# ZhangYY12345/aswStereoMatch

Hardware: AMD Instinct MI355X
Metric: disparity Mpix/s, 1920x1080 D=128 classic bilateral ASW (computeAdaptiveWeight) (higher is better)
Workload: dtype f64; 1 GPU; 1920x1080 D=128 win=15 bilateral, 8 frames/GPU/step resident in HBM, cost volume kept; candidates=129, parallelism=frames sharded, no collective, ranks=1, backend=none

## Files before the change

aswstereomatch_amd/csrc/asw_internal.h:

```cpp
#pragma once
#include <hip/hip_runtime.h>
#include <stddef.h>
#include <stdint.h>

#include <map>
#include <string>
#include <vector>

#include "../../include/asw_mi355x.h"

#define ASW_HIP_TRY(expr)                                  \
    do {                                                   \
        hipError_t _e = (expr);                            \
        if (_e != hipSuccess) {                            \
            asw_note_hip_error(_e, #expr, __FILE__, __LINE__); \
            return ASW_ERR_HIP;                            \
        }                                                  \
    } while (0)

void asw_note_hip_error(hipError_t e, const char* what, const char* file, int line);

struct DevBuf {
    void* p = nullptr;
    size_t cap = 0;
// ... 86 lines not shown
    const uint8_t* gL;
    const uint8_t* gR;
    int H, W, win, minD, nD;
    const int4* taps;
    const float* lut;
    int ntaps;
    int flip;
    float* vol;
    float* disp;
    double* partE;
    float* partD;
    int max_slices;
    int c_begin = 0;
    int resume = 0;
    int out_slice = -1;
};
int bilateral_xq_candidates(int nwave);
constexpr int XQ_LUT_SCALE_LOG2 = 60;
bool bilateral_xq_lut_ok(const float* lut, size_t n);
int launch_bilateral_xq(hipStream_t s, hipStream_t s_border, int nwave, const uint8_t* gL, const uint8_t* gR, int H, int W, int minD,
                        const int4* cells, const float* lut, float* vol, double* bestE, float* bestD, float* disp, bool right = false);
int launch_bilateral(hipStream_t s, const BilateralLaunch& a);
int launch_merge_slices(hipStream_t s, const double* partE, const float* partD, int nz, size_t plane, float* disp);
int bilateral_lds_row_stride(int win);

int launch_scharr_x(hipStream_t s, const uint8_t* img, int H, int W, int pad, short* grad );
size_t similarity_parts_words(int H, int W, int numD);
int launch_similarity(hipStream_t s, const uint8_t* L, const uint8_t* R, const short* gL, const short* gR, int H, int W,
                      int minD, int numD, double regularity, double thresC, double thresG, float* cost, uint32_t* ord_scratch,
                      float2* scales);
int launch_pad_reflect(hipStream_t s, const float* src, int n, int H, int W, int h, float* dst);
int launch_slice_scales(hipStream_t s, const float* vol, int n, size_t plane, uint32_t* ord_scratch , float2* scales);
int launch_u8_scale(hipStream_t s, const uint8_t* img, size_t nbytes, uint32_t* ord_scratch , float2* scale1);
int launch_guide_scales_lr(hipStream_t s, const uint8_t* ref_img, const uint8_t* shifted_img, int H, int W, int minD, int numD,
                           int disp_type, uint32_t* ord_scratch, int* colmm_scratch , float2* scales );

struct NccLaunch {
    const uint8_t* gref;
// ... 151 lines not shown
```

aswstereomatch_amd/csrc/asw_methods.hip:

```cpp
#include <limits.h>
#include <math.h>
#include <stdio.h>
#include <stdlib.h>
#include <string.h>

#include <mutex>
#include <utility>
#include <vector>

#include "asw_internal.h"
#include "asw_host.h"

static int check_direction(int disparity_type)
{
    return disparity_type == ASW_DISPARITY_LEFT || disparity_type == ASW_DISPARITY_RIGHT ? ASW_OK : ASW_ERR_BAD_ARGUMENT;
}

static int ensure_outputs(Frame* f, int planes, bool keep_volume, bool volume_needed = false)
{
    const size_t plane = (size_t)f->rows * f->cols;
    ASW_TRY(f->disp.ensure(plane * 4));
    f->vol_floats = 0;
    if (keep_volume || volume_needed) ASW_TRY(f->vol.ensure(plane * planes * 4));
    if (keep_volume) f->vol_floats = plane * planes;
// ... 164 lines not shown
    a.H = H; a.W = W; a.win = mp.win; a.minD = mp.minD; a.nD = nD;
    a.taps = ctx->bil.taps.as<int4>(); a.lut = ctx->bil.lut.as<float>(); a.ntaps = ctx->bil.ntaps;
    a.vol = keep_volume ? f->vol.as<float>() : nullptr;
    a.disp = f->disp.as<float>();
    a.partE = nullptr; a.partD = nullptr; a.max_slices = 0;
    const bool xq_fits = flip ? (W - 1) / 64 * 64 + mp.minD <= W - 1 : mp.minD <= 48;
    const int xq_waves = nD >= bilateral_xq_candidates(8) ? 8 : 4;
    const bool use_xq = !direct8 && mp.win == 15 && nD >= bilateral_xq_candidates(xq_waves) && mp.minD >= 0 && xq_fits && W >= 64 &&
                        ctx->bil.xq_lut_ok && ctx->tune.bilateral_xq != 0;
    const size_t plane = (size_t)H * W;
    if (use_xq) {
        a.max_slices = 2;
        ASW_TRY(slice_scratch(ctx, a.max_slices, plane, &a.partE, &a.partD));
        a.c_begin = bilateral_xq_candidates(xq_waves);
        const bool tail = nD > a.c_begin;
        ASW_TRY(agg_begin(ctx));
        ASW_HIP_TRY(hipEventRecord(ctx->aux_ev[0], ctx->stream));
        ASW_HIP_TRY(hipStreamWaitEvent(ctx->aux[0], ctx->aux_ev[0], 0));
        ASW_TRY(launch_bilateral_xq(ctx->stream, ctx->aux[0], xq_waves, a.gL, a.gR, H, W, mp.minD, ctx->bil.cells.as<int4>(), ctx->bil.lut_xq.as<float>(), a.vol,
                                    a.partE, a.partD, tail ? nullptr : a.disp, flip != 0));
        ASW_HIP_TRY(hipEventRecord(ctx->aux_ev[1], ctx->aux[0]));
        if (tail) {
            ASW_HIP_TRY(hipStreamWaitEvent(ctx->aux[1], ctx->aux_ev[0], 0));
            a.out_slice = 1;
            ASW_TRY(launch_bilateral(ctx->aux[1], a));
            ASW_HIP_TRY(hipEventRecord(ctx->aux_ev[2], ctx->aux[1]));
            ASW_HIP_TRY(hipStreamWaitEvent(ctx->stream, ctx->aux_ev[2], 0));
        }
        ASW_HIP_TRY(hipStreamWaitEvent(ctx->stream, ctx->aux_ev[1], 0));
        if (tail) ASW_TRY(launch_merge_slices(ctx->stream, a.partE, a.partD, 2, plane, a.disp));
        return agg_end(ctx, tail ? 4 : 2);
    }
    if (plane <= (size_t)1 << 20) {
        a.max_slices = 8;
        ASW_TRY(slice_scratch(ctx, a.max_slices, plane, &a.partE, &a.partD));
    }
    ASW_TRY(agg_begin(ctx));
    ASW_TRY(launch_bilateral(ctx->stream, a));
    return agg_end(ctx, 1);
}

static int run_bilateral_classic(asw_ctx* ctx, Frame* f, const MatchParams& mp, bool keep_volume)
{
    return run_bilateral(ctx, f, mp, keep_volume, false);
}
// ... 724 lines not shown
```

aswstereomatch_amd/csrc/k_bilateral.hip:

```cpp
#include <stdlib.h>

#include <algorithm>
#include <type_traits>

#include "asw_device.h"
#include "asw_internal.h"

namespace {

constexpr int TW = 64;
constexpr int TH = 4;
constexpr int DCMAX = 16;

struct BilParams {
    int H, W, h, minD, nD, ntaps;
    int flip;
    int cand_per_z;
    int c_begin;
    int resume;
    int out_slice;
};

constexpr __host__ __device__ int round_up(int v, int a) { return (v + a - 1) / a * a; }

struct Layout {
    int h, TR, LW, LWp, RW, RWp, offC, offWR, offWL, offL, offR, total;
    __host__ __device__ constexpr Layout(int h_, int G)
        : h(h_), TR(TH + 2 * h_), LW(TW + 2 * h_), LWp(round_up(TW + 2 * h_, 4)), RW(TW + 2 * h_ + DCMAX - 1),
          RWp(round_up(TW + 2 * h_ + DCMAX - 1, 4)), offC(0), offWR(round_up((TH + 2 * h_) * (TW + 2 * h_) * DCMAX, 16)),
          offWL(offWR + round_up(G * TH * (TW + DCMAX - 1) * 4, 16)),
          offL(offWR + round_up(G * TH * (TW + DCMAX - 1) * 4, 16) + G * TH * TW * 4),
          offR(offWR + round_up(G * TH * (TW + DCMAX - 1) * 4, 16) + G * TH * TW * 4 +
               round_up((TH + 2 * h_) * round_up(TW + 2 * h_, 4), 16)),
          total(offWR + round_up(G * TH * (TW + DCMAX - 1) * 4, 16) + G * TH * TW * 4 +
                round_up((TH + 2 * h_) * round_up(TW + 2 * h_, 4), 16) +
// ... 21 lines not shown
}

template <int DC, int G>
__device__ __forceinline__ void process_chunk(const BilParams& p, const uint8_t* __restrict__ gR,
                                              const int4* __restrict__ taps, const float* __restrict__ lut,
                                              float* __restrict__ vol, const Layout& lay, unsigned char* smem, int c0,
                                              double& bestE, float& bestD)
{
    uint8_t* sL = smem + lay.offL;
    uint8_t* sR = smem + lay.offR;
    uint8_t* sC = smem + lay.offC;
    float* sWR = reinterpret_cast<float*>(smem + lay.offWR);
    float* sWL = reinterpret_cast<float*>(smem + lay.offWL);
    constexpr int SWR = TW + DC - 1;
    const int tid = threadIdx.x, tx = tid & 63, ty = tid >> 6;
    const int x0 = blockIdx.x * TW, y0 = blockIdx.y * TH;
    const int H = p.H, W = p.W, h = lay.h, LW = lay.LW, LWp = lay.LWp, RWp = lay.RWp, TR = lay.TR;
    const int RW = TW + 2 * h + DC - 1;
    const int d0 = p.minD + c0;
    const int sRx0 = max(x0 - h - (d0 + DC - 1), -h);

    __syncthreads();
    for (int i = tid; i < TR * RW; i += 256) {
        int r = i / RW, c = i - r * RW;
        int yy = min(max(y0 - h + r, 0), H - 1), xx = min(max(sRx0 + c, 0), W - 1);
        sR[r * RWp + c] = gR[(size_t)yy * W + (p.flip ? W - 1 - xx : xx)];
    }
    __syncthreads();
    const bool interior = x0 - h - (d0 + DC - 1) >= 0 && x0 + TW + h - d0 <= W;
    const bool interiorC = x0 - h - (d0 + DC - 1) >= 0 && x0 + TW + h <= W;
    for (int i = tid; i < TR * LW; i += 256) {
// ... 92 lines not shown
            load_cost<DC>(myC + tp.x * DC, cw);
            const float* w = myWR + t * (TH * SWR);
#pragma unroll
            for (int dd = 0; dd < DC; dd++) {
                float ab = wl * w[-dd];
                double abd = (double)ab;
                double c = (double)(int)((cw[dd >> 2] >> (8 * (dd & 3))) & 0xffu);
                num[dd] = __builtin_fma(abd, c, num[dd]);
                den[dd] = den[dd] + abd;
            }
        }
        wave_lds_sync();
    }

    const int x = x0 + tx, y = y0 + ty;
    if (x < W && y < H) {
#pragma unroll
        for (int dd = 0; dd < DC; dd++) {
            double E = num[dd] / den[dd];
            if (vol) vol[((size_t)(c0 + dd) * H + y) * W + (p.flip ? W - 1 - x : x)] = (float)E;
            if (E < bestE) {
                bestE = E;
                bestD = (float)(d0 + dd);
            }
        }
    }
}

template <int HH, int G, int WPE>
__global__ __launch_bounds__(256) __attribute__((amdgpu_waves_per_eu(WPE, WPE))) void k_asw_bilateral(
    BilParams p, const uint8_t* __restrict__ gL, const uint8_t* __restrict__ gR, const int4* __restrict__ taps,
    const float* __restrict__ lut, float* __restrict__ vol, float* __restrict__ disp, double* __restrict__ partE,
    float* __restrict__ partD)
{
    extern __shared__ __align__(16) unsigned char smem[];
    const Layout lay(HH > 0 ? HH : p.h, G);
    const int tid = threadIdx.x;
    const int x0 = blockIdx.x * TW, y0 = blockIdx.y * TH;
    const int H = p.H, W = p.W, h = lay.h;

    uint8_t* sL = smem + lay.offL;
    for (int i = tid; i < lay.TR * lay.LW; i += 256) {
        int r = i / lay.LW, c = i - r * lay.LW;
        int yy = min(max(y0 - h + r, 0), H - 1), xx = min(max(x0 - h + c, 0), W - 1);
        sL[r * lay.LWp + c] = gL[(size_t)yy * W + (p.flip ? W - 1 - xx : xx)];
    }

    double bestE = 1.7976931348623157e308;
    float bestD = 0.0f;
    if (p.resume) {
        const int xr = x0 + (tid & 63), yr = y0 + (tid >> 6);
        if (xr < W && yr < H) {
            const size_t o = (size_t)yr * W + (p.flip ? W - 1 - xr : xr);
            bestE = partE[o];
            bestD = partD[o];
        }
    }
    int c0 = p.c_begin + blockIdx.z * p.cand_per_z;
    const int cEnd = min(p.nD, c0 + p.cand_per_z);
    for (; c0 + 16 <= cEnd; c0 += 16) process_chunk<16, G>(p, gR, taps, lut, vol, lay, smem, c0, bestE, bestD);
    if (cEnd - c0 >= 8) { process_chunk<8, G>(p, gR, taps, lut, vol, lay, smem, c0, bestE, bestD); c0 += 8; }
    if (cEnd - c0 >= 4) { process_chunk<4, G>(p, gR, taps, lut, vol, lay, smem, c0, bestE, bestD); c0 += 4; }
    if (cEnd - c0 >= 2) { process_chunk<2, G>(p, gR, taps, lut, vol, lay, smem, c0, bestE, bestD); c0 += 2; }
    if (cEnd - c0 >= 1) { process_chunk<1, G>(p, gR, taps, lut, vol, lay, smem, c0, bestE, bestD); c0 += 1; }

    const int x = x0 + (tid & 63), y = y0 + (tid >> 6);
    if (x < W && y < H) {
        const size_t o = (size_t)y * W + (p.flip ? W - 1 - x : x);
        if (gridDim.z == 1 && p.out_slice < 0) {
            disp[o] = bestD;
        } else {
            const int z = gridDim.z == 1 ? p.out_slice : (int)blockIdx.z;
            partE[(size_t)z * H * W + o] = bestE;
            partD[(size_t)z * H * W + o] = bestD;
        }
    }
}

__global__ __launch_bounds__(256) void k_merge_slices(const double* __restrict__ partE, const float* __restrict__ partD, int nz,
                                                      size_t plane, float* __restrict__ disp)
{
    const size_t o = (size_t)blockIdx.x * blockDim.x + threadIdx.x;
    if (o >= plane) return;
    double best = 1.7976931348623157e308;
    float bd = 0.0f;
    for (int z = 0; z < nz; z++) {
        const double e = partE[(size_t)z * plane + o];
        if (e < best) { best = e; bd = partD[(size_t)z * plane + o]; }
    }
    disp[o] = bd;
}

template <int HH, int G, int WPE = 2>
int launch_t(hipStream_t s, const BilateralLaunch& a)
{
    BilParams p;
    p.H = a.H; p.W = a.W; p.h = a.win / 2; p.minD = a.minD; p.nD = a.nD; p.ntaps = a.ntaps; p.flip = a.flip;
    p.c_begin = a.c_begin; p.resume = a.resume; p.out_slice = a.out_slice;
    if (a.c_begin < 0 || a.c_begin >= a.nD || ((a.resume || a.out_slice >= 0) && !(a.partE && a.partD))) return ASW_ERR_BAD_ARGUMENT;
    const Layout lay(p.h, G);
    if (lay.total > 160 * 1024) return ASW_ERR_BAD_ARGUMENT;
    auto kern = k_asw_bilateral<HH, G, WPE>;
    if (lay.total > 64 * 1024)
        ASW_HIP_TRY(hipFuncSetAttribute(reinterpret_cast<const void*>(kern), hipFuncAttributeMaxDynamicSharedMemorySize, lay.total));
    dim3 grid((a.W + TW - 1) / TW, (a.H + TH - 1) / TH);
    if (a.ntaps % G != 0) return ASW_ERR_BAD_ARGUMENT;
    const int tiles = grid.x * grid.y, chunks16 = (a.nD - a.c_begin + 15) / 16;
    int nz = 1;
    if (a.c_begin == 0 && !a.resume && a.out_slice < 0 && a.partE && a.partD && tiles < 2048) nz = std::min(chunks16, std::min(a.max_slices, (2048 + tiles - 1) / tiles));
    const int chunks_per_z = (chunks16 + nz - 1) / nz;
    nz = (chunks16 + chunks_per_z - 1) / chunks_per_z;
    p.cand_per_z = chunks_per_z * 16;
    grid.z = nz;
    hipLaunchKernelGGL(kern, grid, dim3(256), lay.total, s, p, a.gL, a.gR, a.taps, a.lut, a.vol, a.disp, a.partE, a.partD);
    if (nz > 1) {
        const size_t plane = (size_t)a.H * a.W;
        hipLaunchKernelGGL(k_merge_slices, dim3((unsigned)((plane + 255) / 256)), dim3(256), 0, s, a.partE, a.partD, nz, plane, a.disp);
    }
    ASW_HIP_TRY(hipGetLastError());
    return ASW_OK;
}

}

int bilateral_lds_row_stride(int win) { return TW + 2 * (win / 2); }

int launch_merge_slices(hipStream_t s, const double* partE, const float* partD, int nz, size_t plane, float* disp)
{
    hipLaunchKernelGGL(k_merge_slices, dim3((unsigned)((plane + 255) / 256)), dim3(256), 0, s, partE, partD, nz, plane, disp);
    ASW_HIP_TRY(hipGetLastError());
    return ASW_OK;
}

int launch_bilateral(hipStream_t s, const BilateralLaunch& a)
{
    switch (a.win) {
    case 15: return launch_t<7, 4, 4>(s, a);
    case 35: return launch_t<17, 4, 2>(s, a);
    default: return launch_t<0, 4, 3>(s, a);
    }
}
```

aswstereomatch_amd/csrc/k_bilateral_xq.hip:

```cpp
#include <stdlib.h>

#include <algorithm>
#include <cmath>

#include "asw_device.h"
#include "asw_internal.h"

namespace {

constexpr int HH = 7;
constexpr int KS = 2 * HH + 1;
constexpr int PXW = 64;
constexpr int LWC = PXW + 2 * HH;
constexpr int NSTEP = KS + 3;
constexpr int RING = 5;
constexpr int URI = 3;
constexpr int CROW = 6;
static_assert(KS % URI == 0 && CROW % URI == 0, "whole bodies");
constexpr int NCELLCOL = NSTEP + 3;
constexpr int LW8 = 80;
constexpr int LWP = 80;

template <int NW>
struct XqCfg {
// ... 4 lines not shown
    static constexpr int RWC = NPOS + 2 * HH;
    static constexpr int NFIN = 4 * NJ;
    static constexpr int RW8 = (RWC + 3) / 4 * 4;
    static constexpr int NROWS = (KS + NW - 1) / NW;
    static constexpr int RWP = (RWC + 3) / 4 * 4;
    static constexpr int LROW = RING * PXW + LWP;
    static constexpr int RROW = 2 * NPOS + RWP;
    static constexpr int LGRAY = RING * PXW;
    static constexpr int RGRAY = 2 * NPOS;
    static constexpr int OFF_LB = 0;
    static constexpr int OFF_RB = OFF_LB + KS * LROW * 4;
    static constexpr int OFF_L8 = OFF_RB + KS * RROW * 4;
    static constexpr int OFF_R8 = OFF_L8 + KS * LW8;
    static constexpr int OFF_CELL = OFF_R8 + KS * RW8;
    static constexpr int OFF_E64 = 0;
    static constexpr int OFF_PART = NFIN * PXW * 8;
    static constexpr int LDS_TOTAL = std::max((OFF_CELL + NCELLCOL * KS * 2 + 15) / 16 * 16, OFF_PART + NW * PXW * 12);
    static_assert(LDS_TOTAL <= (NW == 8 ? 80 : 53) * 1024, "two (NW = 8) / three (NW = 4) workgroups per CU");
    static_assert(OFF_RB % 16 == 0 && (LROW * 4) % 16 == 0 && (RROW * 4) % 16 == 0 && (NPOS * 4) % 16 == 0 && (LGRAY * 4) % 16 == 0, "b128 alignment");
    static_assert(NPOS % 64 == 0, "positions are staged in whole wavefront passes");
};
#define XQ_CONSTS(NW)                                                                                                           \
    typedef XqCfg<NW> Cfg;                                                                                                       \
    constexpr int NWAVE = Cfg::NWAVE, NTHR = Cfg::NTHR, NJ = Cfg::NJ, NPOS = Cfg::NPOS, RWC = Cfg::RWC, NFIN = Cfg::NFIN, RW8 = Cfg::RW8,      \
                  NROWS = Cfg::NROWS, LROW = Cfg::LROW, RROW = Cfg::RROW, LGRAY = Cfg::LGRAY, RGRAY = Cfg::RGRAY,               \
                  OFF_LB = Cfg::OFF_LB, OFF_RB = Cfg::OFF_RB, OFF_L8 = Cfg::OFF_L8, OFF_R8 = Cfg::OFF_R8, OFF_CELL = Cfg::OFF_CELL,  \
                  LDS_TOTAL = Cfg::LDS_TOTAL, OFF_E64 = Cfg::OFF_E64, OFF_PART = Cfg::OFF_PART;                                  \
    (void)NWAVE; (void)NTHR; (void)NJ; (void)NPOS; (void)RWC; (void)NFIN; (void)RW8; (void)NROWS; (void)LROW; (void)RROW; (void)LGRAY;  \
    (void)RGRAY; (void)OFF_LB; (void)OFF_RB; (void)OFF_L8; (void)OFF_R8; (void)OFF_CELL; (void)LDS_TOTAL; (void)OFF_E64; (void)OFF_PART;

struct XqParams {
// ... 61 lines not shown
        if (Kn < KS) sWL[ky * LROW + lane] = st.v[rr][0];
#pragma unroll
        for (int r3 = 0; r3 < NPOS / 64; r3++) sWR[ky * RROW + lane + 64 * r3] = st.v[rr][1 + r3];
    }
}

template <int NW>
__device__ __forceinline__ void stage_weights(int Kn, const float* __restrict__ lut, unsigned char* smem, int wave, int lane,
                                              uint32_t ppack)
{
    Staged<NW> st;
    stage_issue<NW>(Kn, lut, smem, wave, lane, ppack, st);
    stage_commit<NW>(Kn, smem, wave, lane, st);
}

template <int NW, int K, bool EDGE, bool WRAPW, bool COMMIT, bool RIGHT>
__device__ __forceinline__ void run_step(unsigned char* smem, int g, int qrel, int qrel2, int xabs, int dbase, int dbase2,
                                         int W, int x0, int posmin, double (&num)[4][4], double (&den)[4][4], int wave, int lane,
                                         const Staged<NW>& st)
{
    XQ_CONSTS(NW)
    constexpr int BLO = K > KS - 1 ? K - (KS - 1) : 0;
    constexpr int BHI = K < 3 ? K : 3;
    constexpr int DLO = 0 - BHI, DHI = 3 - BLO;
    const uint32_t* sLd = reinterpret_cast<const uint32_t*>(smem + OFF_LB) + LGRAY;
    const uint32_t* sRd = reinterpret_cast<const uint32_t*>(smem + OFF_RB) + RGRAY;

    int iL[7], iR[7];
    if constexpr (EDGE) {
#pragma unroll
        for (int dl = DLO; dl <= DHI; dl++) {
            const int lc = min(max(xabs + dl + K - HH, 0), W - 1);
            const int rc = RIGHT ? lc + ((dl > 0 ? dbase2 : dbase) - dl) : lc - ((dl < 0 ? dbase2 : dbase) + dl);
            iL[dl + 3] = min(max(lc - (x0 - HH), 0), LWC - 1);
            iR[dl + 3] = min(max(rc - (posmin - HH), 0), RWC - 1);
        }
    }
    typedef __attribute__((address_space(3))) const unsigned char lds_u8;
    lds_u8* bL = (lds_u8*)smem + OFF_LB + 16 * g;
    lds_u8* bR = (lds_u8*)smem + OFF_RB + 4 * qrel;
    lds_u8* bR2 = (lds_u8*)smem + OFF_RB + 4 * qrel2;
    uint32_t hi0[7];
#pragma unroll
    for (int i = 0; i < 7; i++) asm volatile("v_mov_b32 %0, 0" : "=v"(hi0[i]));
    constexpr int UR = EDGE ? 1 : URI;
    auto rows = [&](int ky0, int nbody) {
#pragma unroll 1
        for (int it = 0; it < nbody; it++) {
#pragma unroll
            for (int u = 0; u < UR; u++) {
                lds_u8* rL = bL + u * 4 * LROW;
                lds_u8* rR = bR + u * 4 * RROW;
                lds_u8* rR2 = bR2 + u * 4 * RROW;
                double c[7];
                if constexpr (!EDGE) {
                    const uint32_t gr = *(const __attribute__((address_space(3))) uint32_t*)(rR + 4 * (RGRAY + K));
                    uint32_t gr2 = gr;
                    if constexpr (WRAPW && (RIGHT ? DHI > 0 : DLO < 0)) gr2 = *(const __attribute__((address_space(3))) uint32_t*)(rR2 + 4 * (RGRAY + K));
                    constexpr int E0 = (K + DLO) & ~3, NQ = (K + DHI - E0 + 4) / 4;
                    static_assert(E0 >= 0 && E0 + 4 * NQ + 4 * 15 <= LWP, "the quads stay inside a tile row");
                    typedef uint32_t u32x4 __attribute__((ext_vector_type(4)));
                    const __attribute__((address_space(3))) u32x4* pl4 = (const __attribute__((address_space(3))) u32x4*)(rL + 4 * (LGRAY + E0));
                    uint32_t glv[4 * NQ];
#pragma unroll
                    for (int i = 0; i < NQ; i++) {
                        u32x4 t = pl4[i];
                        asm("" : "+v"(t));
                        glv[4 * i] = t.x; glv[4 * i + 1] = t.y; glv[4 * i + 2] = t.z; glv[4 * i + 3] = t.w;
                    }
#pragma unroll
                    for (int dl = DLO; dl <= DHI; dl++) c[dl + 3] = cost_sample(glv[K + dl - E0], (RIGHT ? dl > 0 : dl < 0) ? gr2 : gr, hi0[dl + 3]);
                } else {
                    const int ky = ky0 + it * UR + u;
#pragma unroll
                    for (int dl = DLO; dl <= DHI; dl++) c[dl + 3] = cost_sample(sLd[ky * LROW + iL[dl + 3]], sRd[ky * RROW + iR[dl + 3]], hi0[dl + 3]);
                }
                typedef float f32x4 __attribute__((ext_vector_type(4)));
                typedef __attribute__((address_space(3))) const f32x4 lds_f32x4;
                const f32x4 wr4 = *(lds_f32x4*)(rR + 4 * (K & 1) * NPOS);
                typedef float f32x2 __attribute__((ext_vector_type(2)));
                f32x2 wrp[2] = {{wr4.x, wr4.y}, {wr4.z, wr4.w}};
                asm("" : "+v"(wrp[1]));
                f32x2 wr2p[2] = {wrp[0], wrp[1]};
                if constexpr ((WRAPW || EDGE) && (RIGHT ? BLO <= 2 : BHI >= 1)) {
                    const f32x4 w2 = *(lds_f32x4*)(rR2 + 4 * (K & 1) * NPOS);
                    wr2p[0] = f32x2{w2.x, w2.y};
// ... 10 lines not shown
                        const bool w0 = RIGHT ? b < a : a < b, w1 = RIGHT ? b < a + 1 : a + 1 < b;
                        const f32x2 s0 = (w0 ? wr2p : wrp)[b >> 1], s1 = (w1 ? wr2p : wrp)[b >> 1];
                        f32x2 wrb;
                        if (w0 == w1) wrb = (b & 1) ? __builtin_shufflevector(s0, s0, 1, 1) : __builtin_shufflevector(s0, s0, 0, 0);
                        else wrb = f32x2{s0[b & 1], s1[b & 1]};
                        const f32x2 pr = wl2 * wrb;
                        ab[a] = pr.x; ab[a + 1] = pr.y;
                    }
#pragma unroll
                    for (int a = 0; a < 4; a++) {
                        const double abd = (double)ab[a];
                        num[a][b] = __builtin_fma(abd, c[a - b + 3], num[a][b]);
                        den[a][b] = den[a][b] + abd;
                    }
                }
#pragma unroll
                for (int b = BLO; b <= BHI; b++)
                    asm volatile("" :: "v"(num[0][b]), "v"(num[1][b]), "v"(num[2][b]), "v"(num[3][b]),
                                       "v"(den[0][b]), "v"(den[1][b]), "v"(den[2][b]), "v"(den[3][b]) : "memory");
                __builtin_amdgcn_sched_barrier(0);
            }
            bL += UR * 4 * LROW;
            bR += UR * 4 * RROW;
            asm("" : "+v"(bL), "+v"(bR));
            if constexpr (WRAPW || EDGE) {
                bR2 += UR * 4 * RROW;
                asm("" : "+v"(bR2));
            }
        }
    };
    if constexpr (COMMIT) {
        rows(0, CROW / UR);
        stage_commit<NW>(K + 1, smem, wave, lane, st);
        rows(CROW, (KS - CROW) / UR);
    } else {
        rows(0, KS / UR);
    }
}

template <int NW, bool EDGE, bool WRAPW, int ABL, bool RIGHT>
__device__ __forceinline__ void run_all_steps(unsigned char* smem, const float* __restrict__ lut, int wave, int lane,
                                              uint32_t ppack, int g, int qrel, int qrel2, int xabs, int dbase, int dbase2,
                                              int W, int x0, int posmin, double (&num)[4][4], double (&den)[4][4])
{
    Staged<NW> st;
#define ASW_XQ_STEP(KK)                                                                                        \
    if (!(ABL & 1) && (KK) + 1 < NSTEP) {                                                                        \
        if constexpr (EDGE) stage_weights<NW>((KK) + 1, lut, smem, wave, lane, ppack);   \
        else stage_issue<NW>((KK) + 1, lut, smem, wave, lane, ppack, st);                      \
    }                                                                                                           \
    run_step<NW, (KK), EDGE, WRAPW, (!EDGE && !(ABL & 1) && (KK) + 1 < NSTEP), RIGHT>(smem, g, qrel, qrel2, xabs, dbase, dbase2, W, x0, posmin, \
                                                                           num, den, wave, lane, st);          \
    if (!(ABL & 2) || (KK) == NSTEP - 1) __syncthreads();
    ASW_XQ_STEP(0) ASW_XQ_STEP(1) ASW_XQ_STEP(2) ASW_XQ_STEP(3) ASW_XQ_STEP(4) ASW_XQ_STEP(5)
    ASW_XQ_STEP(6) ASW_XQ_STEP(7) ASW_XQ_STEP(8) ASW_XQ_STEP(9) ASW_XQ_STEP(10) ASW_XQ_STEP(11)
    ASW_XQ_STEP(12) ASW_XQ_STEP(13) ASW_XQ_STEP(14) ASW_XQ_STEP(15) ASW_XQ_STEP(16) ASW_XQ_STEP(17)
#undef ASW_XQ_STEP
}

template <int NW, bool EDGE, int ABL, bool RIGHT>
__global__ __launch_bounds__(64 * NW) __attribute__((amdgpu_waves_per_eu(NW == 8 ? 4 : 3, NW == 8 ? 4 : 3))) void k_asw_bilateral_xq(
    XqParams p, const uint8_t* __restrict__ gL, const uint8_t* __restrict__ gR, const int4* __restrict__ cells,
    const float* __restrict__ lut, float* __restrict__ vol, double* __restrict__ bestE, float* __restrict__ bestD,
    float* __restrict__ disp)
{
    XQ_CONSTS(NW)
    __shared__ __align__(16) unsigned char smem[LDS_TOTAL];
    const int tid = threadIdx.x, lane = tid & 63, wave = __builtin_amdgcn_readfirstlane(tid >> 6);
    const int H = p.H, W = p.W;
    const int x0 = (p.tile0 + blockIdx.x) * PXW, y = blockIdx.y;
    const int posmin = RIGHT ? x0 + p.minD : x0 - p.minD - 4 * NJ;

    {
        uint8_t* sL8 = smem + OFF_L8;
        uint8_t* sR8 = smem + OFF_R8;
        uint32_t* sLd = reinterpret_cast<uint32_t*>(smem + OFF_LB) + Cfg::LGRAY;
        uint32_t* sRd = reinterpret_cast<uint32_t*>(smem + OFF_RB) + Cfg::RGRAY;
        for (int i = tid; i < KS * LWC; i += NTHR) {
            const int r = i / LWC, c = i - r * LWC;
            const int yy = min(max(y - HH + r, 0), H - 1), xx = min(max(x0 - HH + c, 0), W - 1);
            const int v = gL[(size_t)yy * W + xx];
            sL8[r * LW8 + c] = (uint8_t)v;
            sLd[r * Cfg::LROW + c] = (uint32_t)v;
        }
        for (int i = tid; i < KS * RWC; i += NTHR) {
            const int r = i / RWC, c = i - r * RWC;
            const int yy = min(max(y - HH + r, 0), H - 1), xx = min(max(posmin - HH + c, 0), W - 1);
            const int v = gR[(size_t)yy * W + xx];
            sR8[r * RW8 + c] = (uint8_t)v;
            sRd[r * Cfg::RROW + c] = (uint32_t)v;
        }
        uint16_t* sCell = reinterpret_cast<uint16_t*>(smem + OFF_CELL);
        for (int i = tid; i < NCELLCOL * KS; i += NTHR) {
            const int4 ci = cells[i];
            sCell[i] = (uint16_t)((uint32_t)(ci.x + 8) | ((uint32_t)(ci.y + 8) << 4) | ((uint32_t)(ci.z >> 8) << 8));
        }
    }
    __syncthreads();

    const int g = (lane & 7) | ((lane >> 2) & 8);
    const int jl = 4 * wave + ((lane >> 3) & 3);
    const int qrel = RIGHT ? 4 * g + 4 * jl : 4 * g + 4 * (NJ - jl);
    const int qrel2 = jl == 0 ? (RIGHT ? 4 * g + 4 * NJ : 4 * g) : qrel;
    const int xabs = x0 + 4 * g;
    const int dbase = p.minD + 4 * jl;
    const int dbase2 = jl == 0 ? p.minD + 4 * NJ : dbase;
    const int pclamp_lo = min(max(0 - posmin, 0), NPOS - 1), pclamp_hi = min(max(W - 1 - posmin, 0), NPOS - 1);
    static_assert(NPOS <= 256, "a clamped position fits a byte");
    uint32_t ppack = 0;
#pragma unroll
    for (int r3 = 0; r3 < NPOS / 64; r3++) ppack |= (uint32_t)min(max(lane + 64 * r3, pclamp_lo), pclamp_hi) << (8 * r3);
    asm volatile("" : "+v"(ppack));

    double num[4][4], den[4][4];
#pragma unroll
    for (int a = 0; a < 4; a++)
#pragma unroll
        for (int b = 0; b < 4; b++) { num[a][b] = 0.0; den[a][b] = 0.0; }

    stage_weights<NW>(0, lut, smem, wave, lane, ppack);
    __syncthreads();
    if (EDGE || wave == 0)
        run_all_steps<NW, EDGE, true, ABL, RIGHT>(smem, lut, wave, lane, ppack, g, qrel, qrel2, xabs, dbase, dbase2, W,
                                                   x0, posmin, num, den);
    else
        run_all_steps<NW, EDGE, false, ABL, RIGHT>(smem, lut, wave, lane, ppack, g, qrel, qrel2, xabs, dbase, dbase2, W,
                                                    x0, posmin, num, den);

    int le = lane;
    asm volatile("" : "+v"(le));
    const int ge = (le & 7) | ((le >> 2) & 8), jle = 4 * wave + ((le >> 3) & 3);
    const int cb = 4 * jle, cb2 = jle == 0 ? 4 * NJ : cb;
    double* sE = reinterpret_cast<double*>(smem + OFF_E64);
#pragma unroll
    for (int a = 0; a < 4; a++)
#pragma unroll
        for (int b = 0; b < 4; b++) {
            const int c = RIGHT ? (b < a ? cb2 : cb) + b - a : (a < b ? cb2 : cb) + a - b;
            sE[c * PXW + 4 * ge + a] = __builtin_ldexp(num[a][b], 954) / __builtin_ldexp(den[a][b], -120);
        }
    __syncthreads();
    const int px = lane, part = wave;
    const int x = x0 + px;
    double be = 1.7976931348623157e308;
    float bd = 0.0f;
    if (x < W) {
        for (int c = 16 * part; c < 16 * part + 16; c++) {
            const double E = sE[c * PXW + px];
            if (vol) vol[((size_t)c * H + y) * W + x] = (float)E;
            if (E < be) { be = E; bd = (float)(p.minD + c); }
        }
    }
    double* sPE = reinterpret_cast<double*>(smem + OFF_PART);
    float* sPD = reinterpret_cast<float*>(smem + OFF_PART + NWAVE * PXW * 8);
    sPE[part * PXW + px] = be;
    sPD[part * PXW + px] = bd;
    __syncthreads();
    if (wave == 0 && x < W) {
        double e = 1.7976931348623157e308;
        float d = 0.0f;
#pragma unroll
        for (int q = 0; q < NWAVE; q++) {
            const double eq = sPE[q * PXW + px];
            if (eq < e) { e = eq; d = sPD[q * PXW + px]; }
        }
        if (disp) {
            disp[(size_t)y * W + x] = d;
        } else {
            bestE[(size_t)y * W + x] = e;
            bestD[(size_t)y * W + x] = d;
        }
    }
}

}

int bilateral_xq_candidates(int nwave) { return 16 * nwave; }

bool bilateral_xq_lut_ok(const float* lut, size_t n)
{
    double mn = 0, mx = 0;
    for (size_t i = 0; i < n; i++) {
        const double v = lut[i];
        if (!(v >= 0)) return false;
        if (v > 0 && (mn == 0 || v < mn)) mn = v;
        if (v > mx) mx = v;
    }
    return mn * mn >= std::ldexp(1.0, -68) && mx * mx < std::ldexp(1.0, 128 - 2 * XQ_LUT_SCALE_LOG2 - 1);
}

namespace {
template <int NW>
int launch_xq_t(hipStream_t s, hipStream_t s_border, const uint8_t* gL, const uint8_t* gR, int H, int W, int minD, const int4* cells,
                const float* lut, float* vol, double* bestE, float* bestD, float* disp, bool right)
{
    const int ntiles = (W + PXW - 1) / PXW;
    const dim3 blk(64 * NW);
    if (right) {
        if ((ntiles - 1) * PXW + minD > W - 1) return ASW_ERR_BAD_ARGUMENT;
        XqParams pe{H, W, minD, 0};
        hipLaunchKernelGGL((k_asw_bilateral_xq<NW, true, 0, true>), dim3(1, H), blk, 0, s_border, pe, gL, gR, cells, lut, vol,
                           bestE, bestD, disp);
        if (ntiles > 1) {
            XqParams pi{H, W, minD, 1};
            hipLaunchKernelGGL((k_asw_bilateral_xq<NW, false, 0, true>), dim3(ntiles - 1, H), blk, 0, s, pi, gL, gR, cells, lut,
                               vol, bestE, bestD, disp);
        }
        ASW_HIP_TRY(hipGetLastError());
        return ASW_OK;
    }
    const int n_int = W >= PXW + HH ? std::min(ntiles, (W - PXW - HH) / PXW + 1) : 0;
#ifdef ASW_XQ_ABLATION
    int abl = 0;
    if (const char* e = getenv("ASW_XQ_ABLATE")) abl = atoi(e) & 3;
    auto ki = abl == 0 ? k_asw_bilateral_xq<NW, false, 0, false> : abl == 1 ? k_asw_bilateral_xq<NW, false, 1, false>
            : abl == 2 ? k_asw_bilateral_xq<NW, false, 2, false> : k_asw_bilateral_xq<NW, false, 3, false>;
#else
    auto ki = k_asw_bilateral_xq<NW, false, 0, false>;
#endif
    auto ke = k_asw_bilateral_xq<NW, true, 0, false>;
    if (n_int > 0) {
        XqParams p{H, W, minD, 0};
        hipLaunchKernelGGL(ki, dim3(n_int, H), blk, 0, s, p, gL, gR, cells, lut, vol, bestE, bestD, disp);
    }
    if (ntiles > n_int) {
        XqParams p{H, W, minD, n_int};
        hipLaunchKernelGGL(ke, dim3(ntiles - n_int, H), blk, 0, s_border, p, gL, gR, cells, lut, vol, bestE, bestD, disp);
    }
    ASW_HIP_TRY(hipGetLastError());
    return ASW_OK;
}
}

int launch_bilateral_xq(hipStream_t s, hipStream_t s_border, int nwave, const uint8_t* gL, const uint8_t* gR, int H, int W, int minD,
                        const int4* cells, const float* lut, float* vol, double* bestE, float* bestD, float* disp, bool right)
{
    if (nwave == 8) return launch_xq_t<8>(s, s_border, gL, gR, H, W, minD, cells, lut, vol, bestE, bestD, disp, right);
    if (nwave == 4) return launch_xq_t<4>(s, s_border, gL, gR, H, W, minD, cells, lut, vol, bestE, bestD, disp, right);
    return ASW_ERR_BAD_ARGUMENT;
}
```

Baseline: 242.8 Mpix/s.

## Fold the last disparity candidate into a spare wavefront of interior xq tiles

With D=128 and 8 waves the xq kernel covers 128 candidates, which leaves one leftover candidate. That candidate used to trigger a full-width launch of the generic bilateral kernel plus a full-plane slice merge. Now one wavefront in each interior tile also accumulates the single leftover candidate and writes the final disparity directly. The generic kernel and the merge run only over the border columns. This adds register and LDS work to one wave per tile and a lot of template complexity, in exchange for removing most of the tail kernel and merge traffic.

```diff
diff --git a/aswstereomatch_amd/csrc/asw_internal.h b/aswstereomatch_amd/csrc/asw_internal.h
--- a/aswstereomatch_amd/csrc/asw_internal.h
+++ b/aswstereomatch_amd/csrc/asw_internal.h
@@ -124,14 +124,19 @@
     int c_begin = 0;
     int resume = 0;
     int out_slice = -1;
+    int col_lo = 0, col_hi = -1;
 };
 int bilateral_xq_candidates(int nwave);
 constexpr int XQ_LUT_SCALE_LOG2 = 60;
 bool bilateral_xq_lut_ok(const float* lut, size_t n);
 int launch_bilateral_xq(hipStream_t s, hipStream_t s_border, int nwave, const uint8_t* gL, const uint8_t* gR, int H, int W, int minD,
-                        const int4* cells, const float* lut, float* vol, double* bestE, float* bestD, float* disp, bool right = false);
+                        const int4* cells, const float* lut, float* vol, double* bestE, float* bestD, float* disp, bool right = false,
+                        bool last = false);
+void bilateral_xq_interior_columns(int W, bool right, int* lo, int* hi);
 int launch_bilateral(hipStream_t s, const BilateralLaunch& a);
 int launch_merge_slices(hipStream_t s, const double* partE, const float* partD, int nz, size_t plane, float* disp);
+int launch_merge_slices_cols(hipStream_t s, const double* partE, const float* partD, int nz, int H, int W, int col_lo, int col_hi,
+                             float* disp);
 int bilateral_lds_row_stride(int win);
 
 int launch_scharr_x(hipStream_t s, const uint8_t* img, int H, int W, int pad, short* grad );
diff --git a/aswstereomatch_amd/csrc/asw_methods.hip b/aswstereomatch_amd/csrc/asw_methods.hip
--- a/aswstereomatch_amd/csrc/asw_methods.hip
+++ b/aswstereomatch_amd/csrc/asw_methods.hip
@@ -202,21 +202,27 @@
         ASW_TRY(slice_scratch(ctx, a.max_slices, plane, &a.partE, &a.partD));
         a.c_begin = bilateral_xq_candidates(xq_waves);
         const bool tail = nD > a.c_begin;
+        int ic_lo = 0, ic_hi = 0;
+        bilateral_xq_interior_columns(W, flip != 0, &ic_lo, &ic_hi);
+        const bool last = nD == a.c_begin + 1 && ic_lo < ic_hi;
+        const int bc_lo = flip ? 0 : ic_hi, bc_hi = flip ? ic_lo : W;
         ASW_TRY(agg_begin(ctx));
         ASW_HIP_TRY(hipEventRecord(ctx->aux_ev[0], ctx->stream));
         ASW_HIP_TRY(hipStreamWaitEvent(ctx->aux[0], ctx->aux_ev[0], 0));
         ASW_TRY(launch_bilateral_xq(ctx->stream, ctx->aux[0], xq_waves, a.gL, a.gR, H, W, mp.minD, ctx->bil.cells.as<int4>(), ctx->bil.lut_xq.as<float>(), a.vol,
-                                    a.partE, a.partD, tail ? nullptr : a.disp, flip != 0));
+                                    a.partE, a.partD, tail && !last ? nullptr : a.disp, flip != 0, last));
         ASW_HIP_TRY(hipEventRecord(ctx->aux_ev[1], ctx->aux[0]));
         if (tail) {
             ASW_HIP_TRY(hipStreamWaitEvent(ctx->aux[1], ctx->aux_ev[0], 0));
             a.out_slice = 1;
+            if (last) { a.col_lo = bc_lo; a.col_hi = bc_hi; }
             ASW_TRY(launch_bilateral(ctx->aux[1], a));
             ASW_HIP_TRY(hipEventRecord(ctx->aux_ev[2], ctx->aux[1]));
             ASW_HIP_TRY(hipStreamWaitEvent(ctx->stream, ctx->aux_ev[2], 0));
         }
         ASW_HIP_TRY(hipStreamWaitEvent(ctx->stream, ctx->aux_ev[1], 0));
-        if (tail) ASW_TRY(launch_merge_slices(ctx->stream, a.partE, a.partD, 2, plane, a.disp));
+        if (tail && last) ASW_TRY(launch_merge_slices_cols(ctx->stream, a.partE, a.partD, 2, H, W, bc_lo, bc_hi, a.disp));
+        else if (tail) ASW_TRY(launch_merge_slices(ctx->stream, a.partE, a.partD, 2, plane, a.disp));
         return agg_end(ctx, tail ? 4 : 2);
     }
     if (plane <= (size_t)1 << 20) {
diff --git a/aswstereomatch_amd/csrc/k_bilateral.hip b/aswstereomatch_amd/csrc/k_bilateral.hip
--- a/aswstereomatch_amd/csrc/k_bilateral.hip
+++ b/aswstereomatch_amd/csrc/k_bilateral.hip
@@ -19,6 +19,8 @@
     int c_begin;
     int resume;
     int out_slice;
+    int tile0;
+    int x_lo, x_hi;
 };
 
 constexpr __host__ __device__ int round_up(int v, int a) { return (v + a - 1) / a * a; }
@@ -70,7 +72,7 @@
     float* sWL = reinterpret_cast<float*>(smem + lay.offWL);
     constexpr int SWR = TW + DC - 1;
     const int tid = threadIdx.x, tx = tid & 63, ty = tid >> 6;
-    const int x0 = blockIdx.x * TW, y0 = blockIdx.y * TH;
+    const int x0 = (p.tile0 + blockIdx.x) * TW, y0 = blockIdx.y * TH;
     const int H = p.H, W = p.W, h = lay.h, LW = lay.LW, LWp = lay.LWp, RWp = lay.RWp, TR = lay.TR;
     const int RW = TW + 2 * h + DC - 1;
     const int d0 = p.minD + c0;
@@ -193,7 +195,7 @@
     }
 
     const int x = x0 + tx, y = y0 + ty;
-    if (x < W && y < H) {
+    if (x >= p.x_lo && x < p.x_hi && y < H) {
 #pragma unroll
         for (int dd = 0; dd < DC; dd++) {
             double E = num[dd] / den[dd];
@@ -215,7 +217,7 @@
     extern __shared__ __align__(16) unsigned char smem[];
     const Layout lay(HH > 0 ? HH : p.h, G);
     const int tid = threadIdx.x;
-    const int x0 = blockIdx.x * TW, y0 = blockIdx.y * TH;
+    const int x0 = (p.tile0 + blockIdx.x) * TW, y0 = blockIdx.y * TH;
     const int H = p.H, W = p.W, h = lay.h;
 
     uint8_t* sL = smem + lay.offL;
@@ -244,7 +246,7 @@
     if (cEnd - c0 >= 1) { process_chunk<1, G>(p, gR, taps, lut, vol, lay, smem, c0, bestE, bestD); c0 += 1; }
 
     const int x = x0 + (tid & 63), y = y0 + (tid >> 6);
-    if (x < W && y < H) {
+    if (x >= p.x_lo && x < p.x_hi && y < H) {
         const size_t o = (size_t)y * W + (p.flip ? W - 1 - x : x);
         if (gridDim.z == 1 && p.out_slice < 0) {
             disp[o] = bestD;
@@ -270,6 +272,21 @@
     disp[o] = bd;
 }
 
+__global__ __launch_bounds__(64) void k_merge_slices_cols(const double* __restrict__ partE, const float* __restrict__ partD, int nz,
+                                                          int H, int W, int x_lo, int wc, float* __restrict__ disp)
+{
+    const int c = blockIdx.x * 64 + threadIdx.x;
+    if (c >= wc) return;
+    const size_t plane = (size_t)H * W, o = (size_t)blockIdx.y * W + x_lo + c;
+    double best = 1.7976931348623157e308;
+    float bd = 0.0f;
+    for (int z = 0; z < nz; z++) {
+        const double e = partE[(size_t)z * plane + o];
+        if (e < best) { best = e; bd = partD[(size_t)z * plane + o]; }
+    }
+    disp[o] = bd;
+}
+
 template <int HH, int G, int WPE = 2>
 int launch_t(hipStream_t s, const BilateralLaunch& a)
 {
@@ -277,12 +294,17 @@
     p.H = a.H; p.W = a.W; p.h = a.win / 2; p.minD = a.minD; p.nD = a.nD; p.ntaps = a.ntaps; p.flip = a.flip;
     p.c_begin = a.c_begin; p.resume = a.resume; p.out_slice = a.out_slice;
     if (a.c_begin < 0 || a.c_begin >= a.nD || ((a.resume || a.out_slice >= 0) && !(a.partE && a.partD))) return ASW_ERR_BAD_ARGUMENT;
+    const int c_lo = std::max(a.col_lo, 0), c_hi = a.col_hi < 0 ? a.W : std::min(a.col_hi, a.W);
+    if (c_lo >= c_hi) return ASW_ERR_BAD_ARGUMENT;
+    p.x_lo = a.flip ? a.W - c_hi : c_lo;
+    p.x_hi = a.flip ? a.W - c_lo : c_hi;
+    p.tile0 = p.x_lo / TW;
     const Layout lay(p.h, G);
     if (lay.total > 160 * 1024) return ASW_ERR_BAD_ARGUMENT;
     auto kern = k_asw_bilateral<HH, G, WPE>;
     if (lay.total > 64 * 1024)
         ASW_HIP_TRY(hipFuncSetAttribute(reinterpret_cast<const void*>(kern), hipFuncAttributeMaxDynamicSharedMemorySize, lay.total));
-    dim3 grid((a.W + TW - 1) / TW, (a.H + TH - 1) / TH);
+    dim3 grid((p.x_hi - 1) / TW - p.tile0 + 1, (a.H + TH - 1) / TH);
     if (a.ntaps % G != 0) return ASW_ERR_BAD_ARGUMENT;
     const int tiles = grid.x * grid.y, chunks16 = (a.nD - a.c_begin + 15) / 16;
     int nz = 1;
@@ -311,6 +333,16 @@
     return ASW_OK;
 }
 
+int launch_merge_slices_cols(hipStream_t s, const double* partE, const float* partD, int nz, int H, int W, int col_lo, int col_hi,
+                             float* disp)
+{
+    if (col_lo < 0 || col_hi > W || col_lo >= col_hi) return ASW_ERR_BAD_ARGUMENT;
+    const int wc = col_hi - col_lo;
+    hipLaunchKernelGGL(k_merge_slices_cols, dim3((wc + 63) / 64, H), dim3(64), 0, s, partE, partD, nz, H, W, col_lo, wc, disp);
+    ASW_HIP_TRY(hipGetLastError());
+    return ASW_OK;
+}
+
 int launch_bilateral(hipStream_t s, const BilateralLaunch& a)
 {
     switch (a.win) {
diff --git a/aswstereomatch_amd/csrc/k_bilateral_xq.hip b/aswstereomatch_amd/csrc/k_bilateral_xq.hip
--- a/aswstereomatch_amd/csrc/k_bilateral_xq.hip
+++ b/aswstereomatch_amd/csrc/k_bilateral_xq.hip
@@ -42,7 +42,7 @@
     static constexpr int OFF_R8 = OFF_L8 + KS * LW8;
     static constexpr int OFF_CELL = OFF_R8 + KS * RW8;
     static constexpr int OFF_E64 = 0;
-    static constexpr int OFF_PART = NFIN * PXW * 8;
+    static constexpr int OFF_PART = (NFIN + 1) * PXW * 8;
     static constexpr int LDS_TOTAL = std::max((OFF_CELL + NCELLCOL * KS * 2 + 15) / 16 * 16, OFF_PART + NW * PXW * 12);
     static_assert(LDS_TOTAL <= (NW == 8 ? 80 : 53) * 1024, "two (NW = 8) / three (NW = 4) workgroups per CU");
     static_assert(OFF_RB % 16 == 0 && (LROW * 4) % 16 == 0 && (RROW * 4) % 16 == 0 && (NPOS * 4) % 16 == 0 && (LGRAY * 4) % 16 == 0, "b128 alignment");
@@ -134,11 +134,31 @@
     stage_commit<NW>(Kn, smem, wave, lane, st);
 }
 
-template <int NW, int K, bool EDGE, bool WRAPW, bool COMMIT, bool RIGHT>
+__device__ __forceinline__ int fresh_lane()
+{
+    int l;
+    asm volatile("v_mbcnt_lo_u32_b32 %0, -1, 0\n\tv_mbcnt_hi_u32_b32 %0, -1, %0" : "=&v"(l));
+    return l;
+}
+template <int NPOS>
+__device__ __forceinline__ uint32_t pack_positions(int lane, int pclamp_lo, int pclamp_hi)
+{
+    uint32_t ppack = 0;
+#pragma unroll
+    for (int r3 = 0; r3 < NPOS / 64; r3++) ppack |= (uint32_t)min(max(lane + 64 * r3, pclamp_lo), pclamp_hi) << (8 * r3);
+    asm volatile("" : "+v"(ppack));
+    return ppack;
+}
+template <int NW> constexpr int UWAVE = NW - 1;
+template <bool ON> struct USums {};
+template <> struct USums<true> { double num = 0.0, den = 0.0; };
+
+template <int NW, int K, bool EDGE, bool WRAPW, bool COMMIT, bool RIGHT, bool LASTW, bool FRESH>
 __device__ __forceinline__ void run_step(unsigned char* smem, int g, int qrel, int qrel2, int xabs, int dbase, int dbase2,
-                                         int W, int x0, int posmin, double (&num)[4][4], double (&den)[4][4], int wave, int lane,
-                                         const Staged<NW>& st)
-{
+                                         int W, int x0, int posmin, double (&num)[4][4], double (&den)[4][4], USums<LASTW>& us,
+                                         int wave, int lane, const Staged<NW>& st)
+{
+    static_assert(!LASTW || (!EDGE && !WRAPW), "the last-candidate units live in a plain wavefront of an interior tile");
     XQ_CONSTS(NW)
     constexpr int BLO = K > KS - 1 ? K - (KS - 1) : 0;
     constexpr int BHI = K < 3 ? K : 3;
@@ -160,6 +180,27 @@
     lds_u8* bL = (lds_u8*)smem + OFF_LB + 16 * g;
     lds_u8* bR = (lds_u8*)smem + OFF_RB + 4 * qrel;
     lds_u8* bR2 = (lds_u8*)smem + OFF_RB + 4 * qrel2;
+    lds_u8* uL = nullptr; lds_u8* uW = nullptr; lds_u8* uG = nullptr;
+    if constexpr (FRESH) {
+        static_assert(!EDGE, "interior tiles");
+        const int l2 = fresh_lane();
+        g = (l2 & 7) | ((l2 >> 2) & 8);
+        const int jl = 4 * wave + ((l2 >> 3) & 3);
+        qrel = RIGHT ? 4 * g + 4 * jl : 4 * g + 4 * (NJ - jl);
+        qrel2 = jl == 0 ? (RIGHT ? 4 * g + 4 * NJ : 4 * g) : qrel;
+        bL = (lds_u8*)smem + OFF_LB + 16 * g;
+        bR = (lds_u8*)smem + OFF_RB + 4 * qrel;
+        bR2 = (lds_u8*)smem + OFF_RB + 4 * qrel2;
+    }
+    if constexpr (LASTW) {
+        static_assert(FRESH, "g is this step's own");
+        const int a = (fresh_lane() >> 3) & 3;
+        const int slot = a == 0 ? (K + RING) % RING : a == 1 ? (K - 1 + RING) % RING : a == 2 ? (K - 2 + RING) % RING : (K - 3 + RING) % RING;
+        uL = (lds_u8*)smem + OFF_LB + 16 * g + 4 * a + 4 * PXW * slot;
+        uW = (lds_u8*)smem + OFF_RB + 16 * g + (RIGHT ? 16 * NJ : 0) + 4 * a + 4 * (K & 1) * NPOS;
+        uG = (lds_u8*)smem + OFF_RB + 16 * g + (RIGHT ? 16 * NJ : 0);
+        asm("" : "+v"(uL), "+v"(uW), "+v"(uG));
+    }
     uint32_t hi0[7];
 #pragma unroll
     for (int i = 0; i < 7; i++) asm volatile("v_mov_b32 %0, 0" : "=v"(hi0[i]));
@@ -173,6 +214,8 @@
                 lds_u8* rR = bR + u * 4 * RROW;
                 lds_u8* rR2 = bR2 + u * 4 * RROW;
                 double c[7];
+                uint32_t glU = 0;
+                (void)glU;
                 if constexpr (!EDGE) {
                     const uint32_t gr = *(const __attribute__((address_space(3))) uint32_t*)(rR + 4 * (RGRAY + K));
                     uint32_t gr2 = gr;
@@ -190,6 +233,8 @@
                     }
 #pragma unroll
                     for (int dl = DLO; dl <= DHI; dl++) c[dl + 3] = cost_sample(glv[K + dl - E0], (RIGHT ? dl > 0 : dl < 0) ? gr2 : gr, hi0[dl + 3]);
+                    static_assert(DLO <= 0 && DHI >= 0, "diagonal 0 is in use in every step");
+                    glU = glv[K - E0];
                 } else {
                     const int ky = ky0 + it * UR + u;
 #pragma unroll
@@ -230,6 +275,19 @@
                         den[a][b] = den[a][b] + abd;
                     }
                 }
+                if constexpr (LASTW) {
+                    constexpr int E0 = (K + DLO) & ~3;
+                    (void)E0;
+                    typedef __attribute__((address_space(3))) const uint32_t lds_u32;
+                    typedef __attribute__((address_space(3))) const float lds_f32;
+                    const float wlU = *(lds_f32*)(uL + u * 4 * LROW);
+                    const float wrU = *(lds_f32*)(uW + u * 4 * RROW);
+                    const uint32_t grU = *(lds_u32*)(uG + u * 4 * RROW + 4 * (RGRAY + K));
+                    const double abU = (double)(wlU * wrU);
+                    us.num = __builtin_fma(abU, cost_sample(glU, grU, hi0[3]), us.num);
+                    us.den = us.den + abU;
+                    asm volatile("" :: "v"(us.num), "v"(us.den));
+                }
 #pragma unroll
                 for (int b = BLO; b <= BHI; b++)
                     asm volatile("" :: "v"(num[0][b]), "v"(num[1][b]), "v"(num[2][b]), "v"(num[3][b]),
@@ -243,30 +301,38 @@
                 bR2 += UR * 4 * RROW;
                 asm("" : "+v"(bR2));
             }
+            if constexpr (LASTW) {
+                uL += UR * 4 * LROW;
+                uW += UR * 4 * RROW;
+                uG += UR * 4 * RROW;
+                asm("" : "+v"(uL), "+v"(uW), "+v"(uG));
+            }
         }
     };
     if constexpr (COMMIT) {
         rows(0, CROW / UR);
-        stage_commit<NW>(K + 1, smem, wave, lane, st);
+        stage_commit<NW>(K + 1, smem, wave, FRESH ? fresh_lane() : lane, st);
         rows(CROW, (KS - CROW) / UR);
     } else {
         rows(0, KS / UR);
     }
 }
 
-template <int NW, bool EDGE, bool WRAPW, int ABL, bool RIGHT>
+template <int NW, bool EDGE, bool WRAPW, int ABL, bool RIGHT, bool LASTW = false, bool FRESH = false>
 __device__ __forceinline__ void run_all_steps(unsigned char* smem, const float* __restrict__ lut, int wave, int lane,
                                               uint32_t ppack, int g, int qrel, int qrel2, int xabs, int dbase, int dbase2,
-                                              int W, int x0, int posmin, double (&num)[4][4], double (&den)[4][4])
+                                              int W, int x0, int posmin, double (&num)[4][4], double (&den)[4][4], USums<LASTW>& us, int pclamp_lo = 0,
+                                              int pclamp_hi = 0)
 {
     Staged<NW> st;
 #define ASW_XQ_STEP(KK)                                                                                        \
     if (!(ABL & 1) && (KK) + 1 < NSTEP) {                                                                        \
+        if constexpr (FRESH) { lane = fresh_lane(); ppack = pack_positions<XqCfg<NW>::NPOS>(lane, pclamp_lo, pclamp_hi); }  \
         if constexpr (EDGE) stage_weights<NW>((KK) + 1, lut, smem, wave, lane, ppack);   \
         else stage_issue<NW>((KK) + 1, lut, smem, wave, lane, ppack, st);                      \
     }                                                                                                           \
-    run_step<NW, (KK), EDGE, WRAPW, (!EDGE && !(ABL & 1) && (KK) + 1 < NSTEP), RIGHT>(smem, g, qrel, qrel2, xabs, dbase, dbase2, W, x0, posmin, \
-                                                                           num, den, wave, lane, st);          \
+    run_step<NW, (KK), EDGE, WRAPW, (!EDGE && !(ABL & 1) && (KK) + 1 < NSTEP), RIGHT, LASTW, FRESH>(smem, g, qrel, qrel2, xabs, dbase, dbase2, W, x0, \
+                                                                           posmin, num, den, us, wave, lane, st); \
     if (!(ABL & 2) || (KK) == NSTEP - 1) __syncthreads();
     ASW_XQ_STEP(0) ASW_XQ_STEP(1) ASW_XQ_STEP(2) ASW_XQ_STEP(3) ASW_XQ_STEP(4) ASW_XQ_STEP(5)
     ASW_XQ_STEP(6) ASW_XQ_STEP(7) ASW_XQ_STEP(8) ASW_XQ_STEP(9) ASW_XQ_STEP(10) ASW_XQ_STEP(11)
@@ -274,13 +340,14 @@
 #undef ASW_XQ_STEP
 }
 
-template <int NW, bool EDGE, int ABL, bool RIGHT>
+template <int NW, bool EDGE, int ABL, bool RIGHT, bool LASTC = false>
 __global__ __launch_bounds__(64 * NW) __attribute__((amdgpu_waves_per_eu(NW == 8 ? 4 : 3, NW == 8 ? 4 : 3))) void k_asw_bilateral_xq(
     XqParams p, const uint8_t* __restrict__ gL, const uint8_t* __restrict__ gR, const int4* __restrict__ cells,
     const float* __restrict__ lut, float* __restrict__ vol, double* __restrict__ bestE, float* __restrict__ bestD,
     float* __restrict__ disp)
 {
     XQ_CONSTS(NW)
+    static_assert(!(EDGE && LASTC), "the border tiles cannot host the last-candidate units");
     __shared__ __align__(16) unsigned char smem[LDS_TOTAL];
     const int tid = threadIdx.x, lane = tid & 63, wave = __builtin_amdgcn_readfirstlane(tid >> 6);
     const int H = p.H, W = p.W;
@@ -306,6 +373,13 @@
             sR8[r * RW8 + c] = (uint8_t)v;
             sRd[r * Cfg::RROW + c] = (uint32_t)v;
         }
+        if constexpr (LASTC) {
+            float* sWL = reinterpret_cast<float*>(smem + OFF_LB);
+            for (int i = tid; i < KS * 3 * PXW; i += NTHR) {
+                const int r = i / (3 * PXW), c = i - r * (3 * PXW);
+                sWL[r * Cfg::LROW + 2 * PXW + c] = 0.0f;
+            }
+        }
         uint16_t* sCell = reinterpret_cast<uint16_t*>(smem + OFF_CELL);
         for (int i = tid; i < NCELLCOL * KS; i += NTHR) {
             const int4 ci = cells[i];
@@ -323,10 +397,7 @@
     const int dbase2 = jl == 0 ? p.minD + 4 * NJ : dbase;
     const int pclamp_lo = min(max(0 - posmin, 0), NPOS - 1), pclamp_hi = min(max(W - 1 - posmin, 0), NPOS - 1);
     static_assert(NPOS <= 256, "a clamped position fits a byte");
-    uint32_t ppack = 0;
-#pragma unroll
-    for (int r3 = 0; r3 < NPOS / 64; r3++) ppack |= (uint32_t)min(max(lane + 64 * r3, pclamp_lo), pclamp_hi) << (8 * r3);
-    asm volatile("" : "+v"(ppack));
+    const uint32_t ppack = pack_positions<NPOS>(lane, pclamp_lo, pclamp_hi);
 
     double num[4][4], den[4][4];
 #pragma unroll
@@ -334,14 +405,19 @@
 #pragma unroll
         for (int b = 0; b < 4; b++) { num[a][b] = 0.0; den[a][b] = 0.0; }
 
+    USums<LASTC> us;
+    USums<false> none;
     stage_weights<NW>(0, lut, smem, wave, lane, ppack);
     __syncthreads();
     if (EDGE || wave == 0)
-        run_all_steps<NW, EDGE, true, ABL, RIGHT>(smem, lut, wave, lane, ppack, g, qrel, qrel2, xabs, dbase, dbase2, W,
-                                                   x0, posmin, num, den);
+        run_all_steps<NW, EDGE, true, ABL, RIGHT, false, LASTC>(smem, lut, wave, lane, ppack, g, qrel, qrel2, xabs, dbase, dbase2, W,
+                                                                 x0, posmin, num, den, none, pclamp_lo, pclamp_hi);
+    else if (LASTC && wave == UWAVE<NW>)
+        run_all_steps<NW, EDGE, false, ABL, RIGHT, LASTC, LASTC>(smem, lut, UWAVE<NW>, lane, ppack, g, qrel, qrel2, xabs, dbase, dbase2, W,
+                                                                  x0, posmin, num, den, us, pclamp_lo, pclamp_hi);
     else
-        run_all_steps<NW, EDGE, false, ABL, RIGHT>(smem, lut, wave, lane, ppack, g, qrel, qrel2, xabs, dbase, dbase2, W,
-                                                    x0, posmin, num, den);
+        run_all_steps<NW, EDGE, false, ABL, RIGHT, false, LASTC>(smem, lut, wave, lane, ppack, g, qrel, qrel2, xabs, dbase, dbase2, W,
+                                                                  x0, posmin, num, den, none, pclamp_lo, pclamp_hi);
 
     int le = lane;
     asm volatile("" : "+v"(le));
@@ -355,6 +431,8 @@
             const int c = RIGHT ? (b < a ? cb2 : cb) + b - a : (a < b ? cb2 : cb) + a - b;
             sE[c * PXW + 4 * ge + a] = __builtin_ldexp(num[a][b], 954) / __builtin_ldexp(den[a][b], -120);
         }
+    if constexpr (LASTC)
+        if (wave == UWAVE<NW>) sE[NFIN * PXW + 4 * ge + ((le >> 3) & 3)] = __builtin_ldexp(us.num, 954) / __builtin_ldexp(us.den, -120);
     __syncthreads();
     const int px = lane, part = wave;
     const int x = x0 + px;
@@ -380,7 +458,12 @@
             const double eq = sPE[q * PXW + px];
             if (eq < e) { e = eq; d = sPD[q * PXW + px]; }
         }
-        if (disp) {
+        if constexpr (LASTC) {
+            const double eq = sE[NFIN * PXW + px];
+            if (vol) vol[((size_t)NFIN * H + y) * W + x] = (float)eq;
+            if (eq < e) { e = eq; d = (float)(p.minD + NFIN); }
+        }
+        if (LASTC || disp) {
             disp[(size_t)y * W + x] = d;
         } else {
             bestE[(size_t)y * W + x] = e;
@@ -408,7 +491,7 @@
 namespace {
 template <int NW>
 int launch_xq_t(hipStream_t s, hipStream_t s_border, const uint8_t* gL, const uint8_t* gR, int H, int W, int minD, const int4* cells,
-                const float* lut, float* vol, double* bestE, float* bestD, float* disp, bool right)
+                const float* lut, float* vol, double* bestE, float* bestD, float* disp, bool right, bool last)
 {
     const int ntiles = (W + PXW - 1) / PXW;
     const dim3 blk(64 * NW);
@@ -416,11 +499,15 @@
         if ((ntiles - 1) * PXW + minD > W - 1) return ASW_ERR_BAD_ARGUMENT;
         XqParams pe{H, W, minD, 0};
         hipLaunchKernelGGL((k_asw_bilateral_xq<NW, true, 0, true>), dim3(1, H), blk, 0, s_border, pe, gL, gR, cells, lut, vol,
-                           bestE, bestD, disp);
+                           bestE, bestD, last ? nullptr : disp);
         if (ntiles > 1) {
             XqParams pi{H, W, minD, 1};
-            hipLaunchKernelGGL((k_asw_bilateral_xq<NW, false, 0, true>), dim3(ntiles - 1, H), blk, 0, s, pi, gL, gR, cells, lut,
-                               vol, bestE, bestD, disp);
+            if (last)
+                hipLaunchKernelGGL((k_asw_bilateral_xq<NW, false, 0, true, true>), dim3(ntiles - 1, H), blk, 0, s, pi, gL, gR, cells,
+                                   lut, vol, bestE, bestD, disp);
+            else
+                hipLaunchKernelGGL((k_asw_bilateral_xq<NW, false, 0, true>), dim3(ntiles - 1, H), blk, 0, s, pi, gL, gR, cells, lut,
+                                   vol, bestE, bestD, disp);
         }
         ASW_HIP_TRY(hipGetLastError());
         return ASW_OK;
@@ -437,11 +524,16 @@
     auto ke = k_asw_bilateral_xq<NW, true, 0, false>;
     if (n_int > 0) {
         XqParams p{H, W, minD, 0};
-        hipLaunchKernelGGL(ki, dim3(n_int, H), blk, 0, s, p, gL, gR, cells, lut, vol, bestE, bestD, disp);
+        if (last)
+            hipLaunchKernelGGL((k_asw_bilateral_xq<NW, false, 0, false, true>), dim3(n_int, H), blk, 0, s, p, gL, gR, cells, lut, vol,
+                               bestE, bestD, disp);
+        else
+            hipLaunchKernelGGL(ki, dim3(n_int, H), blk, 0, s, p, gL, gR, cells, lut, vol, bestE, bestD, disp);
     }
     if (ntiles > n_int) {
         XqParams p{H, W, minD, n_int};
-        hipLaunchKernelGGL(ke, dim3(ntiles - n_int, H), blk, 0, s_border, p, gL, gR, cells, lut, vol, bestE, bestD, disp);
+        hipLaunchKernelGGL(ke, dim3(ntiles - n_int, H), blk, 0, s_border, p, gL, gR, cells, lut, vol, bestE, bestD,
+                           last ? nullptr : disp);
     }
     ASW_HIP_TRY(hipGetLastError());
     return ASW_OK;
@@ -449,9 +541,21 @@
 }
 
 int launch_bilateral_xq(hipStream_t s, hipStream_t s_border, int nwave, const uint8_t* gL, const uint8_t* gR, int H, int W, int minD,
-                        const int4* cells, const float* lut, float* vol, double* bestE, float* bestD, float* disp, bool right)
-{
-    if (nwave == 8) return launch_xq_t<8>(s, s_border, gL, gR, H, W, minD, cells, lut, vol, bestE, bestD, disp, right);
-    if (nwave == 4) return launch_xq_t<4>(s, s_border, gL, gR, H, W, minD, cells, lut, vol, bestE, bestD, disp, right);
+                        const int4* cells, const float* lut, float* vol, double* bestE, float* bestD, float* disp, bool right, bool last)
+{
+    if (last && !disp) return ASW_ERR_BAD_ARGUMENT;
+    if (nwave == 8) return launch_xq_t<8>(s, s_border, gL, gR, H, W, minD, cells, lut, vol, bestE, bestD, disp, right, last);
+    if (nwave == 4) return launch_xq_t<4>(s, s_border, gL, gR, H, W, minD, cells, lut, vol, bestE, bestD, disp, right, last);
     return ASW_ERR_BAD_ARGUMENT;
 }
+
+void bilateral_xq_interior_columns(int W, bool right, int* lo, int* hi)
+{
+    const int ntiles = (W + PXW - 1) / PXW;
+    if (right) {
+        *lo = ntiles > 1 ? PXW : W; *hi = W;
+    } else {
+        const int n_int = W >= PXW + HH ? std::min(ntiles, (W - PXW - HH) / PXW + 1) : 0;
+        *lo = 0; *hi = std::min(W, n_int * PXW);
+    }
+}
```

Result: faster. 248.5 Mpix/s, median of 6 (+2.4%).
